# han0110/learn-fhe

Measured on AMD Instinct MI355X. Metric: NTTs/sec at N=2^14 q~60-bit, higher is better.
Workload: dtype u64

## Files before the change

### learn-fhe_amd/csrc/arith.hpp

```cpp
#pragma once
#include <type_traits>

#include "dev_arith.hpp"

namespace fhe {

#define FHE_GLOBAL __attribute__((address_space(1)))
template <class T>
__device__ __forceinline__ const FHE_GLOBAL T *as_global(const T *p) {
    return (const FHE_GLOBAL T *)p;
}
#define FHE_CONST __attribute__((address_space(4)))
template <class T>
__device__ __forceinline__ const FHE_CONST T *as_const(const T *p) {
    return (const FHE_CONST T *)p;
}

#define FHE_HEADER_KERNEL static __attribute__((unused)) __global__

template <int I, int END, typename F>
__device__ __forceinline__ void static_for(F &&f) {
    if constexpr (I < END) {
        f(std::integral_constant<int, I>{});
        static_for<I + 1, END>(f);
    }
}

struct ModDesc {
    u64 q;
    const TwPair *tw, *twi;
    u64 ninv[20], ninv_s[20];
    u64 ninv_w[20], ninv_w_s[20];
    u64 one_s;
    const u64 *tww, *twwi;
    unsigned pm_c;
    int pm_b;
    const uint4 *twd, *twdi;
    unsigned ds_pow;
    uint4 ds_ninv[20], ds_ninv_w[20], ds_one;
    const uint4 *twd3i;
    unsigned twd3_stride;
    u64 bar_mu;
    int bar_sh1, bar_sh2;
};

struct NttIo {
    const u64 *src = nullptr;
    unsigned src_mod = 1;
    const u64 *mul = nullptr;
    unsigned mul_div = 1, mul_period = 1;
    const u64 *src2 = nullptr, *src3 = nullptr, *src4 = nullptr;
    unsigned src_group = 0;
    u64 *dst2 = nullptr;
    unsigned dst_period = 0, dst_first2 = 0;
};
__device__ __forceinline__ const u64 *ntt_src(const NttIo &io, unsigned sub, int log_len, const u64 *own) {
    if (!io.src) return own;
    if (io.src_group) {
        const unsigned gsel = sub / io.src_group, r = sub - gsel * io.src_group;
        const u64 *b = gsel == 0 ? io.src : gsel == 1 ? io.src2 : gsel == 2 ? io.src3 : io.src4;
        return b + (size_t(r) << log_len);
    }
    return io.src + (size_t(sub % io.src_mod) << log_len);
}

struct ArithShoup {
    typedef u64 Elem;
    struct K {
        u64 q, q2;
        const FHE_CONST TwPair *tw, *twi;
        u64 ninv, ninv_s;
        int pb, prefix;
        TwPair ninv_w;
        Barrett bar;
    };
    static __device__ __forceinline__ K make(const ModDesc &D, int log_n_total, int pb, int prefix) {
        return K{D.q, 2 * D.q, as_const(D.tw), as_const(D.twi), pb ? 1 : D.ninv[log_n_total], pb ? D.one_s : D.ninv_s[log_n_total], pb, prefix,
                 TwPair{D.ninv_w[log_n_total], D.ninv_w_s[log_n_total]}, Barrett{D.q, D.bar_mu, D.bar_sh1, D.bar_sh2}};
    }
    static __device__ __forceinline__ u64 mulvar(u64 x, u64 y, const K &k) { return mulmod_barrett(x, y, k.bar); }
    template <int PH = 1>
    static __device__ __forceinline__ void gs_last_scaled(u64 &X, u64 &Y, const K &k) {
        const u64 s = X + Y, d = X - Y + k.q2;
        X = csub(mul_shoup_lazy(s, k.ninv, k.ninv_s, k.q), k.q);
        Y = csub(mul_shoup_lazy(d, k.ninv_w.w, k.ninv_w.ws, k.q), k.q);
    }
    template <int PH = 1>
    static __device__ __forceinline__ void gs_last_plain(u64 &X, u64 &Y, const TwPair &p, const K &k) {
        gs_bfly(X, Y, p.w, p.ws, k.q, k.q2);
        X = csub(X, k.q); Y = csub(Y, k.q);
    }
    typedef TwPair TwRaw;
    typedef TwPair TwReg;
    static constexpr int PREFETCH = 0;
    template <bool INV>
    static __device__ __forceinline__ TwRaw fetch(const K &k, int idx) {
        const FHE_CONST TwPair *p = (INV ? k.twi : k.tw) + idx;
// ... 390 lines not shown
        u128 b[32] = {};
        for (int r = 0; r < 32; ++r) b[r] = s.diag.out[r & 7];
        x32(b);
        int g = 3;
        for (int l = 3; l >= 0; --l) layer(s, b, g++, 4, l, 2, 16, false);
        x21(b);
        for (int l = 3; l >= 0; --l) layer(s, b, g++, 4, l, 2, 16, false);
        if (!x10(b, R0, pairs)) s.ok = false;
        for (int l = R0 - 1; l >= 1; --l) layer(s, b, g++, R0, l, 32 >> R0, 1 << R0, false);
        layer(s, b, g++, R0, 0, 32 >> R0, 1 << R0, true);
        s.layers = g;
        return s;
    }
    template <int R0, bool PAIRS, int IN>
    static constexpr Sched SCHED = make(R0, PAIRS, IN);
    template <int R0, bool PAIRS, int IN> static constexpr bool fx(int g, int o) { return SCHED<R0, PAIRS, IN>.lay[g - 3][o].fx; }
    template <int R0, bool PAIRS, int IN> static constexpr bool fy(int g, int o) { return SCHED<R0, PAIRS, IN>.lay[g - 3][o].fy; }
    template <int R0, bool PAIRS, int IN> static constexpr bool fs(int g, int o) { return SCHED<R0, PAIRS, IN>.lay[g - 3][o].fs; }
    template <int R0, bool PAIRS, int IN> static constexpr int mi(int g, int o) {
        return SCHED<R0, PAIRS, IN>.mi(SCHED<R0, PAIRS, IN>.lay[g - 3][o].m);
    }
    template <int R0, bool PAIRS, int IN> static constexpr bool valid() {
        constexpr Sched s = SCHED<R0, PAIRS, IN>;
        return s.ok && s.layers == 11 + R0 && s.bflies == 16 * (11 + R0);
    }
    template <int R0, bool PAIRS, int IN> static constexpr int folds_x100() { return SCHED<R0, PAIRS, IN>.folds * 100 / SCHED<R0, PAIRS, IN>.bflies; }

    static_assert(keep_ok(RMAX), "a raw product must be able to enter a butterfly as it stands");
    static_assert(fold_max(CAP - 1) < 2 * QMIN, "a folded value is below 2q: one conditional subtraction makes it canonical");
    static_assert(cover(RMAX) == L::K, "the offset of a raw subtrahend is DsLazy's K");
    static_assert(valid<1, true, 0>() && valid<2, true, 0>() && valid<3, true, 0>() && valid<4, false, 0>(), "whole rings, canonical inputs");
    static_assert(valid<1, true, 1>() && valid<2, true, 1>() && valid<3, true, 1>() && valid<4, false, 1>(), "multiplied inputs");
    static_assert(valid<1, false, 0>() && valid<2, false, 0>() && valid<3, false, 0>() && valid<3, false, 1>(), "the 8-byte dealing");
};
static_assert(DsGsLazy<60>::SCHED<3, true, 0>.diag.folds == 3 && DsGsLazy<60>::folds_x100<3, true, 0>() <= 75, "60 bits");
static_assert(DsGsLazy<60>::folds_x100<3, true, 1>() <= 75 && DsGsLazy<60>::folds_x100<4, false, 0>() <= 75, "60 bits");
static_assert(DsGsLazy<55>::SCHED<3, true, 0>.diag.folds == 0 && DsGsLazy<55>::folds_x100<3, true, 0>() <= 30, "55 bits");
static_assert(DsGsLazy<54>::SCHED<3, true, 0>.diag.folds == 0 && DsGsLazy<54>::folds_x100<3, true, 0>() <= 30, "54 bits");

template <int B>
struct ArithDS {
    typedef u64 Elem;
    static constexpr u64 MASK = (u64(1) << B) - 1;
    static constexpr int SPLIT = B - 31;
    typedef uint4 TwRaw;
    typedef uint4 TwReg;
    struct K {
        DsK m;
        const FHE_CONST uint4 *tw, *twi;
        uint4 ninv, ninv_w;
        int pb, prefix;
        const FHE_CONST uint4 *tw3i;
        unsigned tw3_stride;
    };
    static constexpr int PREFETCH = 4;
    static __host__ __device__ __forceinline__ uint4 split(u64 w, u64 q) {
        const u64 w1 = (u64)((((unsigned __int128)w) << 32) % q);
        const u64 lo = (u64(1) << SPLIT) - 1;
        return uint4{(unsigned)(w & lo), (unsigned)(w >> SPLIT), (unsigned)(w1 & lo), (unsigned)(w1 >> SPLIT)};
    }
    template <bool INV>
    static __device__ __forceinline__ TwRaw fetch(const K &k, int idx) {
        const FHE_CONST uint4 *p = (INV ? k.twi : k.tw) + idx;
        TwRaw r;
        r.x = p->x; r.y = p->y; r.z = p->z; r.w = p->w;
        return r;
    }
    static __device__ __forceinline__ TwReg prep(const TwRaw &r) { return r; }
    static __device__ __forceinline__ K make(const ModDesc &D, int log_n_total, int pb, int prefix) {
        K k;
        k.m.q = D.q; k.m.q2 = 2 * D.q; k.m.q4 = 4 * D.q;
        k.m.c = D.pm_c; k.m.c2 = 2 * D.pm_c; k.m.pw = D.ds_pow;
        k.m.qk = Lazy::K * D.q;
        asm("" : "+s"(k.m.qk));
        k.tw = as_const(D.twd); k.twi = as_const(D.twdi);
        k.ninv = pb ? D.ds_one : D.ds_ninv[log_n_total];
        k.ninv_w = D.ds_ninv_w[log_n_total];
        k.pb = pb; k.prefix = prefix;
        k.tw3i = as_const(D.twd3i); k.tw3_stride = D.twd3_stride;
        return k;
    }
    typedef DsLazy<B> Lazy;
    static __host__ __device__ __forceinline__ u64 mul_raw(u64 y, const uint4 &w, const DsK &m, u64 add = 0) {
        const unsigned y0 = (unsigned)y, y1 = (unsigned)(y >> 32);
        const u64 s1 = (u64)w.y * y0 + (u64)w.w * y1;
        const u64 s0 = ((u64)w.x * y0 + add) + (u64)w.z * y1;
        const u64 v = (u64)(unsigned)s1 * m.pw + s0;
        return (u64)(unsigned)(s1 >> 32) * m.c2 + v;
    }
    static __host__ __device__ __forceinline__ u64 fold1(u64 x, const DsK &m) {
        const unsigned hi = (unsigned)(x >> 32), h = hi >> (B - 32);
        const u64 base = ((u64)(hi & (unsigned)(MASK >> 32)) << 32) | (unsigned)x;
        return (u64)h * m.c + base;
    }
    static __device__ __forceinline__ u64 mul(u64 y, const uint4 &w, const DsK &m) { return fold1(mul_raw(y, w, m), m); }
    static __device__ __forceinline__ u64 mulvar(u64 x, u64 y, const K &k) {
        return pm_mul<B>(x, ArithPM<B>::split(y), PmK{k.m.q, k.m.q2, k.m.q4, k.m.c, k.m.c2});
    }
    static __device__ __forceinline__ void ct(u64 &X, u64 &Y, const TwReg &w, const K &k) {
        const u64 t = mul(Y, w, k.m);
        const u64 x = X;
        X = x + t;
        Y = x + k.m.q2 - t;
    }
    template <bool FOLDX>
    static __host__ __device__ __forceinline__ void ct_lazy(u64 &X, u64 &Y, const TwReg &w, const DsK &m) {
        const u64 x = FOLDX ? fold1(X, m) : X;
        const u64 r = mul_raw(Y, w, m, x);
        X = r;
        Y = ((x << 1) + m.qk) - r;
    }
    static constexpr int CT_LAYERS = 64;
    static constexpr bool PASS_FOLD = false;
    static constexpr int CT_SPAN = B >= 64 - 2 ? 1 : (((1 << (64 - B)) - 2) / 2 > 64 ? 64 : ((1 << (64 - B)) - 2) / 2);
    static __device__ constexpr bool ct_fold_at(int layer) { return layer > 0 && layer % CT_SPAN == 0; }
    template <int PH>
    static __device__ __forceinline__ void gs(u64 &X, u64 &Y, const TwReg &w, const K &k) {
        static_assert(PH < 64 - B - 1, "sums overflow");
        const u64 s = X + Y;
        const u64 d = X + (k.m.q2 << PH) - Y;
        X = s;
        Y = mul(d, w, k.m);
    }
    static constexpr bool GS_FOLDS = true;
    static constexpr int GS_SPAN = 64 - B - 1 > 8 ? 8 : 64 - B - 1;
    template <int PH = 1>
    static __device__ __forceinline__ void gs_last_scaled(u64 &X, u64 &Y, const K &k) {
        const u64 s = X + Y, d = X + (k.m.q2 << PH) - Y;
        X = csub(mul(s, k.ninv, k.m), k.m.q);
        Y = csub(mul(d, k.ninv_w, k.m), k.m.q);
    }
    template <int PH = 1>
// ... 52 lines not shown
        v[4] = mul_raw((u0 + ou2) - u2, e[3], m); used(3, v[4]);
        v[5] = mul_raw((u1 + ou3) - u3, e[4], m); used(4, v[5]);
        v[6] = mul_raw((e0 + orr) - e2, e[5], m); used(5, v[6]);
        v[7] = mul_raw((e1 + orr) - e3, e[6], m); used(6, v[7]);
    }
    typedef typename ArithPM<B>::MacAcc MacAcc;
    static constexpr int MAC_TERMS = ArithPM<B>::MAC_TERMS;
    static __device__ __forceinline__ PmK pmk(const K &k) { return PmK{k.m.q, k.m.q2, k.m.q4, k.m.c, k.m.c2}; }
    static __device__ __forceinline__ MacAcc mac_zero() { return MacAcc{0, 0}; }
    static __device__ __forceinline__ u64 mac_in(u64 x, const K &) { return x; }
    static __device__ __forceinline__ MacAcc mac(MacAcc acc, u64 xin, u64 kval, int term, const K &k, const Barrett &) {
        const unsigned wl = (unsigned)kval;
        const PmTw w{wl, wl << (63 - B), (unsigned)(kval >> 32)};
        u64 v, u;
        pm_mul_vu<B>(xin, w, v, u);
        acc.v += v; acc.u += u;
        if ((term % MAC_TERMS) == MAC_TERMS - 1) acc = MacAcc{pm_reduce_vu<B>(acc.v, acc.u, pmk(k)), 0};
        return acc;
    }
    static __device__ __forceinline__ u64 mac_finish(MacAcc acc, const K &k) { return pm_reduce_vu<B>(acc.v, acc.u, pmk(k)); }
};

#define FHE_SCHED_FENCE() asm volatile("" ::: "memory")

template <int L0_, int R_, int l_, int REP0_, int NREP_, int STRIDE_, bool SHARED_, int REP_SHIFT_ = 0>
struct Unit {
    static constexpr int L0 = L0_, R = R_, l = l_, REP0 = REP0_, NREP = NREP_, STRIDE = STRIDE_, REP_SHIFT = REP_SHIFT_;
    static constexpr bool SHARED = SHARED_;
    static constexpr int NT = (SHARED_ ? 1 : NREP_) << l_;
    static constexpr int half = 1 << (R_ - 1 - l_);
};

#ifdef FHE_LAB_ABLATE
template <class A, class = void> struct tw_skip_mask { static constexpr unsigned value = 0; };
template <class A> struct tw_skip_mask<A, decltype((void)A::SKIP_MASK)> { static constexpr unsigned value = A::SKIP_MASK; };
#endif

template <class A, bool INV, class U, int NTW>
__device__ __forceinline__ void tw_load(typename A::TwRaw (&raw)[NTW], int top, const typename A::K &k) {
    static_assert(U::NT <= NTW, "twiddle buffer too small for this unit");
#pragma unroll
    for (int rr = 0; rr < (U::SHARED ? 1 : U::NREP); ++rr)
#pragma unroll
        for (int b = 0; b < (1 << U::l); ++b) {
            const int tp = U::SHARED ? top : (top | ((U::REP0 + rr) << U::REP_SHIFT));
            const int idx = (1 << (U::L0 + U::l + k.pb)) + ((((k.prefix << U::L0) | tp)) << U::l) + b;
#ifdef FHE_LAB_ABLATE
            if constexpr ((tw_skip_mask<A>::value >> (U::L0 + U::l)) & 1) { raw[(rr << U::l) | b] = A::fake(k, idx); continue; }
#endif
            raw[(rr << U::l) | b] = A::template fetch<INV>(k, idx);
        }
}

template <class A, class U, int NTW, int E>
__device__ __forceinline__ void ct_apply(typename A::Elem (&x)[E], const typename A::TwRaw (&raw)[NTW], const typename A::K &k) {
    if constexpr ((U::l > 0 && U::l % A::CT_LAYERS == 0) || A::ct_fold_at(U::L0 + U::l)) {
#pragma unroll
        for (int rr = 0; rr < U::NREP; ++rr)
#pragma unroll
            for (int r = 0; r < (1 << U::R); ++r) x[(U::REP0 + rr) * U::STRIDE + r] = A::fold(x[(U::REP0 + rr) * U::STRIDE + r], k);
    }
    if constexpr (U::SHARED) {
#pragma unroll
        for (int b = 0; b < (1 << U::l); ++b) {
            const typename A::TwReg w = A::prep(raw[b]);
#pragma unroll
            for (int rr = 0; rr < U::NREP; ++rr)
#pragma unroll
                for (int j = 0; j < U::half; ++j) {
                    const int o = (U::REP0 + rr) * U::STRIDE + b * 2 * U::half + j;
                    A::ct(x[o], x[o + U::half], w, k);
                }
        }
    } else {
#pragma unroll
        for (int rr = 0; rr < U::NREP; ++rr)
#pragma unroll
            for (int b = 0; b < (1 << U::l); ++b) {
                const typename A::TwReg w = A::prep(raw[(rr << U::l) | b]);
#pragma unroll
                for (int j = 0; j < U::half; ++j) {
                    const int o = (U::REP0 + rr) * U::STRIDE + b * 2 * U::half + j;
                    A::ct(x[o], x[o + U::half], w, k);
                }
            }
    }
}

template <class A, class U, int NTW, int E>
__device__ __forceinline__ void ct_apply_lazy(typename A::Elem (&x)[E], const typename A::TwRaw (&raw)[NTW], const typename A::K &k) {
    constexpr bool FOLDX = A::Lazy::fold_before(U::L0 + U::l);
    constexpr int LAZY_GROUP = 4;
    static_for<0, (U::SHARED ? (1 << U::l) : U::NREP)>([&](auto oc) {
        constexpr int outer = decltype(oc)::value;
        static_for<0, (U::SHARED ? U::NREP : (1 << U::l))>([&](auto ic) {
            constexpr int inner = decltype(ic)::value;
            constexpr int b = U::SHARED ? outer : inner, rr = U::SHARED ? inner : outer;
            const typename A::TwReg w = A::prep(raw[U::SHARED ? b : ((rr << U::l) | b)]);
#pragma unroll
            for (int j = 0; j < U::half; ++j) {
                const int o = (U::REP0 + rr) * U::STRIDE + b * 2 * U::half + j;
                A::template ct_lazy<FOLDX>(x[o], x[o + U::half], w, k.m);
                if ((j + 1) % LAZY_GROUP == 0 || j + 1 == U::half) __builtin_amdgcn_sched_barrier(0);
            }
        });
    });
// ... 78 lines not shown
```

### learn-fhe_amd/csrc/ctx.hpp

```cpp
#pragma once
#include <hip/hip_runtime.h>

#include <cstdint>
#include <vector>

#include "dev_arith.hpp"
#include "modmath.hpp"
#include "ntt_kernels.hpp"

struct fhe_ctx {
    uint64_t q = 0;
    int s = 0;
    uint64_t g = 0;
    uint64_t omega = 0;
    int log_cap = 0;
    std::vector<uint64_t> tw, twi;
    uint64_t ninv[32] = {0}, ninv_s[32] = {0};
    uint64_t ninv_w[32] = {0}, ninv_w_s[32] = {0};
    fhe::Barrett barrett{};
    int device = -1;
    fhe::TwPair *d_tw = nullptr, *d_twi = nullptr;
    u64 *d_tww = nullptr, *d_twwi = nullptr;
    uint4 *d_twd = nullptr, *d_twdi = nullptr;
    uint4 *d_twd3i = nullptr;
    int pm_b = 0;
    unsigned pm_c = 0;
    fhe::ModDesc *d_desc = nullptr;
    fhe::ModDesc h_desc{};
};

namespace fhe {
constexpr int MAX_LOG_N = 17;
int ctx_build_host(uint64_t q, fhe_ctx *c);
int ntt_fwd_multi(const ModDesc *descs, unsigned n_desc, u64 *a, int log_n, size_t batch, hipStream_t st, int pm = 0, NttIo io = NttIo());
int ntt_inv_multi(const ModDesc *descs, unsigned n_desc, u64 *a, int log_n, size_t batch, hipStream_t st, int pm = 0, NttIo io = NttIo());
int ntt_mul_multi(const ModDesc *descs, unsigned n_desc, u64 *a, int log_n, size_t batch, hipStream_t st, int pm, NttIo io);
int ntt_fwd_inner15(const ModDesc *descs, unsigned n_desc, u64 *a, size_t batch, hipStream_t st, int pm, NttIo io = NttIo());
int ntt_inv_inner15(const ModDesc *descs, unsigned n_desc, u64 *a, size_t batch, hipStream_t st, int pm, NttIo io = NttIo());
}
```

### learn-fhe_amd/csrc/ntt14w.hpp

```cpp
#pragma once
#include <type_traits>
#include "ntt_kernels.hpp"

namespace fhe {
namespace w14 {

constexpr int WSLOTS = 1088;
template <int R0> constexpr int threads() { return 64 << R0; }
template <int R0> constexpr size_t lds_bytes() { return (size_t(1) << R0) * WSLOTS * 8; }
constexpr int THREADS = threads<3>();
constexpr size_t LDS_BYTES = lds_bytes<3>();

__device__ __forceinline__ void wave_sync() {
    __builtin_amdgcn_wave_barrier();
    asm volatile("" ::: "memory");
}

template <class A, class = void> struct w14_old_deal { static constexpr bool value = false; };
template <class A> struct w14_old_deal<A, decltype((void)A::W14_OLD_DEAL)> { static constexpr bool value = true; };
template <class A, int R0>
__device__ __host__ constexpr bool w14_pairs() {
    return R0 <= 3 && !w14_old_deal<A>::value;
}

// ... 179 lines not shown
    for (int h = 0; h < 2; ++h) {
#pragma unroll
        for (int r4 = 0; r4 < 16; ++r4) wp[4 * r4] = x[((r4 & 1) << 4) | (h << 3) | (r4 >> 1)];
        wave_sync();
#pragma unroll
        for (int n4 = 0; n4 < 16; ++n4) y[(h << 4) | n4] = rp[68 * n4];
        wave_sync();
    }
#pragma unroll
    for (int r = 0; r < 32; ++r) x[r] = y[r];
}

__device__ __forceinline__ void xchg_23(u64 (&x)[32], int lane, u64 *wl) {
    const int hi5 = ((lane >> 4) << 3) | ((lane & 3) << 1) | ((lane >> 3) & 1);
    u64 *wp = wl + 34 * hi5 + ((lane >> 2) & 1);
    const u64 *rp = wl + 34 * (lane >> 5) + 2 * (lane & 15) + ((lane >> 4) & 1);
    u64 y[32];
#pragma unroll
    for (int h = 0; h < 2; ++h) {
#pragma unroll
        for (int c = 0; c < 16; ++c) wp[2 * c] = x[(h << 4) | c];
        wave_sync();
#pragma unroll
        for (int R = 0; R < 16; ++R)
            y[((R >> 2) << 3) | (h << 2) | (R & 3)] = rp[68 * R];
        wave_sync();
    }
#pragma unroll
    for (int r = 0; r < 32; ++r) x[r] = y[r];
}

__device__ __forceinline__ void xchg_32(u64 (&x)[32], int lane, u64 *wl) {
    const u64 *rp = wl + 17 * lane;
    u64 *wp = wl + 68 * (lane >> 4) + (lane & 15);
    u64 y[32];
#pragma unroll
    for (int h = 0; h < 2; ++h) {
#pragma unroll
        for (int R = 0; R < 16; ++R) wp[17 * (((R >> 2) << 4) | (R & 3))] = x[((R >> 2) << 3) | (h << 2) | (R & 3)];
        wave_sync();
#pragma unroll
        for (int c = 0; c < 16; ++c) y[(h << 4) | c] = rp[c];
        wave_sync();
    }
#pragma unroll
    for (int r = 0; r < 32; ++r) x[r] = y[r];
}

template <int R0, int l> using P0 = Unit<0, R0, l, 0, (32 >> R0), (1 << R0), true>;
template <int R0, int l> using P1 = Unit<R0, 4, l, 0, 2, 16, true>;
template <int R0, int l> using P2 = Unit<R0 + 4, 4, l, 0, 2, 16, true>;
template <int R0, int l, int AB> using P3 = Unit<R0 + 8, 3, l, AB, 1, 8, false, 6>;

template <class A>
__device__ __host__ constexpr bool w14_p3_refill() {
    return std::is_same<typename A::TwRaw, uint4>::value;
}

template <class A>
struct Tw7 {
    typename A::TwRaw l0[1], l1[2], l2[4];
};
template <class A, bool INV, int R0, int AB>
__device__ __forceinline__ void tw7_load(Tw7<A> &b, int t3, const typename A::K &k) {
    tw_load<A, INV, P3<R0, 0, AB>>(b.l0, t3, k);
    tw_load<A, INV, P3<R0, 1, AB>>(b.l1, t3, k);
    tw_load<A, INV, P3<R0, 2, AB>>(b.l2, t3, k);
}

template <int R0, bool PAIRS>
__device__ __forceinline__ void load_p0(u64 (&x)[32], const u64 *__restrict__ g, int t) {
#pragma unroll
    for (int r = 0; r < 32; ++r) {
        const int n = r & ((1 << R0) - 1), pass = r >> R0;
        if constexpr (PAIRS) {
            if (pass & 1) continue;
            const ulonglong2 v = *reinterpret_cast<const ulonglong2 *>(g + ((n << 11) | ((pass >> 1) << (7 + R0)) | (t << 1)));
            x[r] = v.x; x[r + (1 << R0)] = v.y;
        } else {
            x[r] = g[(n << 11) | (pass << (6 + R0)) | t];
        }
    }
}
template <int AB>
__device__ __forceinline__ void load_p3(u64 (&x)[32], const u64 *__restrict__ src) {
#pragma unroll
    for (int j = 0; j < 8; j += 2) {
        const ulonglong2 v = *reinterpret_cast<const ulonglong2 *>(src + (AB << 9) + j);
        x[AB * 8 + j] = v.x; x[AB * 8 + j + 1] = v.y;
    }
}
template <class A, int AB>
__device__ __forceinline__ void load_mul_p3(u64 (&x)[32], const u64 *__restrict__ src, const u64 *__restrict__ mul, const typename A::K &k) {
#pragma unroll
    for (int j = 0; j < 8; j += 2) {
        const ulonglong2 v = *reinterpret_cast<const ulonglong2 *>(src + (AB << 9) + j);
        const ulonglong2 m = *reinterpret_cast<const ulonglong2 *>(mul + (AB << 9) + j);
        x[AB * 8 + j] = A::mulvar(v.x, m.x, k); x[AB * 8 + j + 1] = A::mulvar(v.y, m.y, k);
    }
}

template <class A, int AB>
__device__ __forceinline__ void store_p3(u64 (&x)[32], u64 *__restrict__ dst_wave, int lane, u64 *wl, const typename A::K &k) {
    ulonglong2 *wr = reinterpret_cast<ulonglong2 *>(wl + 8 * lane + (lane & ~1));
    const ulonglong2 *rd = reinterpret_cast<const ulonglong2 *>(wl + 2 * lane + 2 * (lane >> 3));
#pragma unroll
    for (int j = 0; j < 4; ++j) {
        ulonglong2 v;
        v.x = A::canon_fwd(x[AB * 8 + 2 * j], k);
        v.y = A::canon_fwd(x[AB * 8 + 2 * j + 1], k);
        wr[j] = v;
    }
    wave_sync();
#pragma unroll
    for (int kk = 0; kk < 4; ++kk) {
        const ulonglong2 v = rd[72 * kk];
        x[AB * 8 + 2 * kk] = v.x; x[AB * 8 + 2 * kk + 1] = v.y;
    }
    wave_sync();
#pragma unroll
    for (int kk = 0; kk < 4; ++kk) {
        ulonglong2 v;
        v.x = x[AB * 8 + 2 * kk]; v.y = x[AB * 8 + 2 * kk + 1];
        *reinterpret_cast<ulonglong2 *>(dst_wave + (AB << 9) + 128 * kk + 2 * lane) = v;
    }
}

template <class A, int R0, bool KEEP = false>
__device__ __forceinline__ void fwd_one(u64 (&x)[32], u64 *__restrict__ g, const typename A::K &k, u64 *lds, u64 *wl,
                                        const int t, const int lane, const int w STAMP_ENTRY_PARAM) {
    typedef typename A::TwRaw Tw;
    constexpr bool LAZY = w14_lazy_fwd<A, KEEP>();
    if constexpr (LAZY) static_assert(A::Lazy::canon_ok(11 + R0), "lazy outputs of this many layers do not fit canon_fwd");
    STAMP_DECL;
    STAMP_REAL(10);
    STAMP(0);
    {
        Tw a0[1], a1[2], a2[4], a3[8];
        tw_load<A, false, P0<R0, 0>>(a0, 0, k);
        if constexpr (R0 >= 2) tw_load<A, false, P0<R0, (R0 >= 2 ? 1 : 0)>>(a1, 0, k);
        if constexpr (R0 >= 3) tw_load<A, false, P0<R0, (R0 >= 3 ? 2 : 0)>>(a2, 0, k);
        if constexpr (R0 == 4) tw_load<A, false, P0<R0, (R0 == 4 ? 3 : 0)>>(a3, 0, k);
        STAMP(1);
        FHE_SCHED_FENCE();
        w14_ct<LAZY, A, P0<R0, 0>>(x, a0, k);
        if constexpr (R0 >= 2) {
            FHE_SCHED_FENCE();
            w14_ct<LAZY, A, P0<R0, (R0 >= 2 ? 1 : 0)>>(x, a1, k);
        }
        if constexpr (R0 >= 3) {
            FHE_SCHED_FENCE();
            w14_ct<LAZY, A, P0<R0, (R0 >= 3 ? 2 : 0)>>(x, a2, k);
        }
        if constexpr (R0 == 4) {
            FHE_SCHED_FENCE();
            w14_ct<LAZY, A, P0<R0, (R0 == 4 ? 3 : 0)>>(x, a3, k);
        }
    }
    FHE_SCHED_FENCE();
    Tw b0[1], b1[2], b2[4], b3[8];
    tw_load<A, false, P1<R0, 0>>(b0, w, k); tw_load<A, false, P1<R0, 1>>(b1, w, k); tw_load<A, false, P1<R0, 2>>(b2, w, k); tw_load<A, false, P1<R0, 3>>(b3, w, k);
    STAMP(2);
    xchg_01<R0, w14_pairs<A, R0>()>(x, t, w, lds);
    STAMP(3);
    if constexpr (A::PASS_FOLD) {
#pragma unroll
        for (int r = 0; r < 32; ++r) x[r] = A::fold(x[r], k);
    }
    FHE_SCHED_FENCE();
    w14_ct<LAZY, A, P1<R0, 0>>(x, b0, k);
    FHE_SCHED_FENCE();
    w14_ct<LAZY, A, P1<R0, 1>>(x, b1, k);
    FHE_SCHED_FENCE();
    w14_ct<LAZY, A, P1<R0, 2>>(x, b2, k);
    FHE_SCHED_FENCE();
    w14_ct<LAZY, A, P1<R0, 3>>(x, b3, k);
    FHE_SCHED_FENCE();
    const int t2 = (w << 4) | (lane >> 2), t3e = (w << 8) | lane;
    Tw c0[1], c1[2], c2[4], c3[8];
    tw_load<A, false, P2<R0, 0>>(c0, t2, k); tw_load<A, false, P2<R0, 1>>(c1, t2, k); tw_load<A, false, P2<R0, 2>>(c2, t2, k);
    STAMP(4);
    xchg_12(x, lane, wl);
    STAMP(5);
    if constexpr (A::PASS_FOLD) {
#pragma unroll
        for (int r = 0; r < 32; ++r) x[r] = A::fold(x[r], k);
    }
    FHE_SCHED_FENCE();
    w14_ct<LAZY, A, P2<R0, 0>>(x, c0, k);
    FHE_SCHED_FENCE();
    w14_ct<LAZY, A, P2<R0, 1>>(x, c1, k);
    FHE_SCHED_FENCE();
    tw_load<A, false, P2<R0, 3>>(c3, t2, k);
    w14_ct<LAZY, A, P2<R0, 2>>(x, c2, k);
    FHE_SCHED_FENCE();
    w14_ct<LAZY, A, P2<R0, 3>>(x, c3, k);
    FHE_SCHED_FENCE();
    int lane3 = lane, t3 = t3e;
    if constexpr (LAZY) {
        lane3 = __builtin_amdgcn_mbcnt_hi(~0u, __builtin_amdgcn_mbcnt_lo(~0u, 0u));
        asm volatile("" : "+v"(lane3));
        t3 = (w << 8) | lane3;
    }
    Tw7<A> d[2];
    tw7_load<A, false, R0, 0>(d[0], t3, k);
    STAMP(6);
    xchg_23(x, lane3, wl);
    STAMP(7);
    if constexpr (A::PASS_FOLD) {
#pragma unroll
        for (int r = 0; r < 32; ++r) x[r] = A::fold(x[r], k);
    }
    u64 *dst_wave = g + (w << 11);
    static_for<0, 4>([&](auto abc) {
        constexpr int ab = decltype(abc)::value;
        FHE_SCHED_FENCE();
        w14_ct<LAZY, A, P3<R0, 0, ab>>(x, d[ab & 1].l0, k);
        w14_ct<LAZY, A, P3<R0, 1, ab>>(x, d[ab & 1].l1, k);
        FHE_SCHED_FENCE();
        if constexpr (ab < 3) tw7_load<A, false, R0, (ab < 3 ? ab + 1 : 3)>(d[(ab + 1) & 1], t3, k);
        w14_ct<LAZY, A, P3<R0, 2, ab>>(x, d[ab & 1].l2, k);
        FHE_SCHED_FENCE();
        if constexpr (KEEP) {
#pragma unroll
            for (int j = 0; j < 8; ++j) x[ab * 8 + j] = A::canon_fwd(x[ab * 8 + j], k);
        } else {
            store_p3<A, ab>(x, dst_wave, lane3, wl, k);
        }
    });
    STAMP(8);
#ifdef NTT14_STAMPS
    asm volatile("s_waitcnt vmcnt(0)" ::: "memory");
#endif
    STAMP(9);
    STAMP_REAL(11);
    STAMP_FLUSH();
}

template <class A>
__device__ __host__ constexpr bool w14_p3_diag() {
    return std::is_same<typename A::TwRaw, uint4>::value;
}

template <class A, int R0, int AB>
__device__ __forceinline__ int p3_blk(int t3, const typename A::K &k) {
    return (1 << (R0 + 8 + k.pb)) + ((k.prefix << (R0 + 8)) | t3 | (AB << 6));
}
template <class A, int R0, int AB>
__device__ __forceinline__ void p3_diag_load(uint4 (&e)[7], int t3, const typename A::K &k) {
    const int blk = p3_blk<A, R0, AB>(t3, k);
#pragma unroll
    for (int p = 0; p < 7; ++p) {
        const FHE_CONST uint4 *q = k.tw3i + size_t(p) * k.tw3_stride + blk;
        e[p] = uint4{q->x, q->y, q->z, q->w};
    }
}
template <class A, int R0, int AB, int NEXT>
__device__ __forceinline__ void p3_diag_apply(u64 (&x)[32], uint4 (&e)[7], const uint4 &ci, const uint4 &cj, const uint4 &cij, int t3,
                                              const typename A::K &k) {
    const auto &m = k.m;
    u64 *v = x + 8 * AB;
    const u64 s0 = v[0] + v[1], t0 = v[0] + m.q2 - v[1];
    const u64 s1 = v[2] + v[3], t1 = A::mul(v[2] + m.q2 - v[3], ci, m);
    const u64 s2 = v[4] + v[5], t2 = A::mul(v[4] + m.q2 - v[5], cj, m);
    const u64 s3 = v[6] + v[7], t3v = A::mul(v[6] + m.q2 - v[7], cij, m);
    const u64 u0 = s0 + s1, e0 = s0 + m.q4 - s1;
    const u64 u1 = t0 + t1, e1 = t0 + m.q2 - t1;
    const u64 u2 = s2 + s3, e2 = A::mul(s2 + m.q4 - s3, ci, m);
    const u64 u3 = t2 + t3v, e3 = A::mul(t2 + m.q2 - t3v, ci, m);
    const int blk = NEXT >= 0 ? p3_blk<A, R0, (NEXT >= 0 ? NEXT : 0)>(t3, k) : 0;
    auto refill = [&](int p) {
        if constexpr (NEXT >= 0) {
            const FHE_CONST uint4 *q = k.tw3i + size_t(p) * k.tw3_stride + blk;
// ... 30 lines not shown
    if constexpr (LZ) p3_diag_apply_lazy<A, SEL, R0, AB, NEXT>(x, e, ci, cj, cij, t3, k, off);
    else p3_diag_apply<A, R0, AB, NEXT>(x, e, ci, cj, cij, t3, k);
}

template <class A, bool PFX, int R0, int IN, bool LZ>
__device__ __forceinline__ void inv_one(u64 (&x)[32], Tw7<A> (&d)[2], u64 *__restrict__ g, const typename A::K &k, u64 *lds, u64 *wl,
                                        const int t, const int lane, const int w STAMP_ENTRY_PARAM) {
    typedef typename A::TwRaw Tw;
    int t2 = 0;
    if constexpr (!LZ) t2 = (w << 4) | (lane >> 2);
    const int t3 = (w << 8) | lane;
    typedef GsSel<R0, w14_pairs<A, R0>(), IN> SEL;
    u64 off[W14_OFFS] = {};
    if constexpr (LZ) {
        static_assert(w14_p3_diag<A>(), "the lazy inverse is written for the diagonal form of pass 3");
        static_assert(A::GsLazy::template valid<R0, w14_pairs<A, R0>(), IN>(), "no valid lazy schedule");
        w14_gs_offs<A, SEL>(off, k);
    }
    STAMP_DECL;
    STAMP_REAL(10);
    STAMP(0);
    constexpr bool REFILL = w14_p3_refill<A>();
    Tw c3[8], c2[4], c1[2], c0[1];
    if constexpr (w14_p3_diag<A>()) {
        uint4(&e)[7] = reinterpret_cast<uint4(&)[7]>(d[0]);
        const uint4 ci = A::template fetch<true>(k, 1), cj = A::template fetch<true>(k, 2), cij = A::template fetch<true>(k, 3);
        FHE_SCHED_FENCE();
        w14_p3<LZ, A, SEL, R0, 0, 1>(x, e, ci, cj, cij, t3, k, off);
        FHE_SCHED_FENCE();
        w14_p3<LZ, A, SEL, R0, 1, 2>(x, e, ci, cj, cij, t3, k, off);
        FHE_SCHED_FENCE();
        w14_p3<LZ, A, SEL, R0, 2, 3>(x, e, ci, cj, cij, t3, k, off);
        FHE_SCHED_FENCE();
        w14_p3<LZ, A, SEL, R0, 3, -1>(x, e, ci, cj, cij, t3, k, off);
    } else
    static_for<0, 4>([&](auto abc) {
        constexpr int ab = decltype(abc)::value, nx = ab < 3 ? ab + 1 : 3;
        Tw7<A> &e = d[REFILL ? 0 : ab & 1];
        FHE_SCHED_FENCE();
        gs_apply<A, P3<R0, 2, ab>, 0>(x, e.l2, k);
        if constexpr (REFILL && ab < 3) tw_load<A, true, P3<R0, 2, nx>>(e.l2, t3, k);
        FHE_SCHED_FENCE();
        gs_apply<A, P3<R0, 1, ab>, 1>(x, e.l1, k);
        if constexpr (REFILL && ab < 3) tw_load<A, true, P3<R0, 1, nx>>(e.l1, t3, k);
        gs_apply<A, P3<R0, 0, ab>, 2>(x, e.l0, k);
        if constexpr (REFILL && ab < 3) tw_load<A, true, P3<R0, 0, nx>>(e.l0, t3, k);
        FHE_SCHED_FENCE();
        if constexpr (!REFILL && ab < 2) tw7_load<A, true, R0, (ab < 2 ? ab + 2 : 3)>(d[ab & 1], t3, k);
    });
    FHE_SCHED_FENCE();
    STAMP(1);
    if constexpr (LZ) t2 = (w << 4) | (lane >> 2);
    constexpr bool C3_LATE = sizeof(Tw) > 8;
    if constexpr (!C3_LATE) tw_load<A, true, P2<R0, 3>>(c3, t2, k);
    xchg_32(x, lane, wl);
    STAMP(2);
    FHE_SCHED_FENCE();
    if constexpr (C3_LATE) tw_load<A, true, P2<R0, 3>>(c3, t2, k);
    constexpr bool C2_LATE = LZ;
    if constexpr (!C2_LATE) tw_load<A, true, P2<R0, 2>>(c2, t2, k);
    if constexpr (LZ) w14_gs_offs<A, SEL>(off, k);
    w14_gs<LZ, A, P2<R0, 3>, SEL, 3>(x, c3, k, off);
    FHE_SCHED_FENCE();
    if constexpr (C2_LATE) tw_load<A, true, P2<R0, 2>>(c2, t2, k);
    tw_load<A, true, P2<R0, 1>>(c1, t2, k); tw_load<A, true, P2<R0, 0>>(c0, t2, k);
    w14_gs<LZ, A, P2<R0, 2>, SEL, 4>(x, c2, k, off);
    FHE_SCHED_FENCE();
    w14_gs<LZ, A, P2<R0, 1>, SEL, 5>(x, c1, k, off);
    FHE_SCHED_FENCE();
    w14_gs<LZ, A, P2<R0, 0>, SEL, 6>(x, c0, k, off);
    FHE_SCHED_FENCE();
    STAMP(3);
    Tw b3[8], b2[4], b1[2], b0[1];
    tw_load<A, true, P1<R0, 3>>(b3, w, k); tw_load<A, true, P1<R0, 2>>(b2, w, k); tw_load<A, true, P1<R0, 1>>(b1, w, k); tw_load<A, true, P1<R0, 0>>(b0, w, k);
    xchg_21(x, lane, wl);
    STAMP(4);
    FHE_SCHED_FENCE();
    if constexpr (LZ) w14_gs_offs<A, SEL>(off, k);
    w14_gs<LZ, A, P1<R0, 3>, SEL, 7>(x, b3, k, off);
    FHE_SCHED_FENCE();
    w14_gs<LZ, A, P1<R0, 2>, SEL, 8>(x, b2, k, off);
    FHE_SCHED_FENCE();
    w14_gs<LZ, A, P1<R0, 1>, SEL, 9>(x, b1, k, off);
    FHE_SCHED_FENCE();
    w14_gs<LZ, A, P1<R0, 0>, SEL, 10>(x, b0, k, off);
    FHE_SCHED_FENCE();
    STAMP(5);
    Tw a3[8], a2[4], a1[2], a0[1];
    if constexpr (R0 == 4) tw_load<A, true, P0<R0, (R0 == 4 ? 3 : 0)>>(a3, 0, k);
    if constexpr (R0 >= 3) tw_load<A, true, P0<R0, (R0 >= 3 ? 2 : 0)>>(a2, 0, k);
    if constexpr (R0 >= 2) tw_load<A, true, P0<R0, (R0 >= 2 ? 1 : 0)>>(a1, 0, k);
    if constexpr (PFX) tw_load<A, true, P0<R0, 0>>(a0, 0, k);
    xchg_10<R0, w14_pairs<A, R0>()>(x, t, w, lds);
    STAMP(6);
    if constexpr (LZ) w14_gs_offs<A, SEL>(off, k);
    if constexpr (R0 == 4) {
        FHE_SCHED_FENCE();
        w14_gs<LZ, A, P0<R0, (R0 == 4 ? 3 : 0)>, SEL, 11>(x, a3, k, off);
    }
    if constexpr (R0 >= 3) {
        FHE_SCHED_FENCE();
        w14_gs<LZ, A, P0<R0, (R0 >= 3 ? 2 : 0)>, SEL, 8 + R0>(x, a2, k, off);
    }
    if constexpr (R0 >= 2) {
        FHE_SCHED_FENCE();
        w14_gs<LZ, A, P0<R0, (R0 >= 2 ? 1 : 0)>, SEL, 9 + R0>(x, a1, k, off);
    }
    STAMP(7);
    typename A::TwReg wlast{};
    if constexpr (PFX) wlast = A::prep(a0[0]);
    constexpr int LAST_PH = A::GS_SPAN > 0 ? (10 + R0) % (A::GS_SPAN > 0 ? A::GS_SPAN : 1) : 1;
    constexpr int HALF = 1 << (R0 - 1), REPS = 32 >> R0, CH = HALF < 4 ? HALF : 4;
    constexpr bool PAIRS = w14_pairs<A, R0>();
    constexpr int CHP = CH < 2 ? 1 : CH / 2;
    if constexpr (LZ) {
        w14_gs_offs<A, SEL>(off, k);
        auto last = [&](auto oc) {
            typedef typename A::GsLazy G;
// ... 199 lines not shown
```

### learn-fhe_amd/csrc/ring_api.hip

```cpp
#include <hip/hip_runtime.h>
#include <cstdlib>

#include <cstring>
#include <mutex>
#include <new>
#include <set>
#include <utility>

#include "../../include/fhe_ring.h"
#include "api_common.hpp"
#include "ctx.hpp"
#include "dispatch.hpp"
#include "ntt_kernels.hpp"
#include "ntt14w.hpp"

using fhe::u64;

namespace {
int check_transform(const fhe_ctx *ctx, const void *a, size_t n, size_t batch) {
    if (!ctx || !is_pow2(n) || (!a && batch)) return FHE_ERR_INVALID;
    if (n == 1) return FHE_OK;
    int log_n = ilog2(n);
    if (log_n > ctx->s - 1) return FHE_ERR_NO_ROOT;
    if (log_n > ctx->log_cap) return FHE_ERR_UNSUPPORTED;
// ... 227 lines not shown
    if (!c) return FHE_ERR_INVALID;
    int rc = fhe::ctx_build_host(q, c);
    if (rc != FHE_OK) { delete c; return rc; }
    c->device = device;
    if (device >= 0) {
        DeviceGuard guard(device);
        if (!guard.ok) { delete c; return FHE_ERR_HIP; }
        const size_t cap = c->tw.size();
        std::vector<fhe::TwPair> pf(cap), pi(cap);
        for (size_t j = 0; j < cap; ++j) {
            pf[j] = {c->tw[j], fhe::shoup(c->tw[j], q)};
            pi[j] = {c->twi[j], fhe::shoup(c->twi[j], q)};
        }
        hipError_t e = hipMalloc(&c->d_tw, cap * sizeof(fhe::TwPair));
        if (e == hipSuccess) e = hipMalloc(&c->d_twi, cap * sizeof(fhe::TwPair));
        if (e == hipSuccess) e = hipMemcpy(c->d_tw, pf.data(), cap * sizeof(fhe::TwPair), hipMemcpyHostToDevice);
        if (e == hipSuccess) e = hipMemcpy(c->d_twi, pi.data(), cap * sizeof(fhe::TwPair), hipMemcpyHostToDevice);
        if (e == hipSuccess && c->pm_b) {
            const int b = c->pm_b;
            std::vector<uint64_t> lf(cap), li(cap);
            auto pack = [b](uint64_t w) { return ((w >> (b - 31)) << 32) | (w & ((uint64_t(1) << (b - 31)) - 1)); };
            for (size_t j = 0; j < cap; ++j) { lf[j] = pack(c->tw[j]); li[j] = pack(c->twi[j]); }
            e = hipMalloc((void **)&c->d_tww, 2 * cap * sizeof(uint64_t));
            c->d_twwi = c->d_tww + cap;
            if (e == hipSuccess) e = hipMemcpy(c->d_tww, lf.data(), cap * sizeof(uint64_t), hipMemcpyHostToDevice);
            if (e == hipSuccess) e = hipMemcpy(c->d_twwi, li.data(), cap * sizeof(uint64_t), hipMemcpyHostToDevice);
        }
        if (e == hipSuccess && c->pm_b) {
            const int b = c->pm_b;
            std::vector<uint4> df(cap), di(cap);
            auto split = [b, q](uint64_t w) {
                const uint64_t w1 = (uint64_t)((((unsigned __int128)w) << 32) % q), lo = (uint64_t(1) << (b - 31)) - 1;
                return uint4{(unsigned)(w & lo), (unsigned)(w >> (b - 31)), (unsigned)(w1 & lo), (unsigned)(w1 >> (b - 31))};
            };
            for (size_t j = 0; j < cap; ++j) { df[j] = split(c->tw[j]); di[j] = split(c->twi[j]); }
            for (int k = 0; k < 20; ++k) { c->h_desc.ds_ninv[k] = split(c->ninv[k]); c->h_desc.ds_ninv_w[k] = split(c->ninv_w[k]); }
            c->h_desc.ds_one = split(1);
            e = hipMalloc((void **)&c->d_twd, 2 * cap * sizeof(uint4));
            c->d_twdi = c->d_twd + cap;
            if (e == hipSuccess) e = hipMemcpy(c->d_twd, df.data(), cap * sizeof(uint4), hipMemcpyHostToDevice);
            if (e == hipSuccess) e = hipMemcpy(c->d_twdi, di.data(), cap * sizeof(uint4), hipMemcpyHostToDevice);
            if (e == hipSuccess && cap >= 8) {
                const size_t stride = cap / 4;
                std::vector<uint4> d3(7 * stride, uint4{0, 0, 0, 0});
                for (size_t blk = 1; blk < stride; ++blk) {
                    const uint64_t th = c->twi[4 * blk];
                    uint64_t pw = th;
                    for (int p = 0; p < 7; ++p) { d3[p * stride + blk] = split(pw); pw = fhe::mulmod(pw, th, q); }
                }
                e = hipMalloc((void **)&c->d_twd3i, d3.size() * sizeof(uint4));
                if (e == hipSuccess) e = hipMemcpy(c->d_twd3i, d3.data(), d3.size() * sizeof(uint4), hipMemcpyHostToDevice);
                c->h_desc.twd3i = c->d_twd3i; c->h_desc.twd3_stride = (unsigned)stride;
            }
        }
        c->h_desc.tww = c->d_tww;
        c->h_desc.twwi = c->d_twwi;
        c->h_desc.twd = c->d_twd;
        c->h_desc.twdi = c->d_twdi;
        c->h_desc.ds_pow = c->pm_b ? 1u << (c->pm_b - 31) : 0;
        c->h_desc.pm_b = c->pm_b;
        c->h_desc.pm_c = c->pm_c;
        c->h_desc.q = q;
        c->h_desc.tw = c->d_tw;
        c->h_desc.twi = c->d_twi;
        for (int k = 0; k < 20; ++k) {
            c->h_desc.ninv[k] = c->ninv[k]; c->h_desc.ninv_s[k] = c->ninv_s[k];
            c->h_desc.ninv_w[k] = c->ninv_w[k]; c->h_desc.ninv_w_s[k] = c->ninv_w_s[k];
        }
        c->h_desc.one_s = fhe::shoup(1, q);
        c->h_desc.bar_mu = c->barrett.mu; c->h_desc.bar_sh1 = c->barrett.sh1; c->h_desc.bar_sh2 = c->barrett.sh2;
        if (e == hipSuccess) e = hipMalloc(&c->d_desc, sizeof(fhe::ModDesc));
        if (e == hipSuccess) e = hipMemcpy(c->d_desc, &c->h_desc, sizeof(fhe::ModDesc), hipMemcpyHostToDevice);
        if (e != hipSuccess) {
            g_last_hip = (int)e;
            fhe_ctx_destroy(c);
            return FHE_ERR_HIP;
        }
    }
    *out = c;
    return FHE_OK;
}

void fhe_ctx_destroy(fhe_ctx *c) {
    if (!c) return;
    if (c->device >= 0) {
        DeviceGuard guard(c->device);
        if (c->d_tw) (void)hipFree(c->d_tw);
        if (c->d_twi) (void)hipFree(c->d_twi);
        if (c->d_desc) (void)hipFree(c->d_desc);
        if (c->d_tww) (void)hipFree(c->d_tww);
        if (c->d_twd) (void)hipFree(c->d_twd);
        if (c->d_twd3i) (void)hipFree(c->d_twd3i);
    }
    delete c;
}

int fhe_ctx_info(const fhe_ctx *c, uint64_t *q, int *s, uint64_t *g, uint64_t *omega) {
    if (!c) return FHE_ERR_INVALID;
    if (q) *q = c->q;
    if (s) *s = c->s;
    if (g) *g = c->g;
    if (omega) *omega = c->omega;
    return FHE_OK;
}

int fhe_ctx_twiddles(const fhe_ctx *c, int inverse, uint64_t *out, size_t count) {
    if (!c || !out) return FHE_ERR_INVALID;
    const auto &t = inverse ? c->twi : c->tw;
    if (count > t.size()) return FHE_ERR_UNSUPPORTED;
    std::memcpy(out, t.data(), count * sizeof(uint64_t));
    return FHE_OK;
}

static int transform_entry(const fhe_ctx *ctx, uint64_t *a, size_t n, size_t batch, fhe_mem mem, void *stream, bool inverse) {
    int rc = check_transform(ctx, a, n, batch);
    if (rc != FHE_OK) return rc;
    if (ctx->device < 0) return FHE_ERR_NO_DEVICE;
    if (n == 1 || batch == 0) return FHE_OK;
    if (batch > 0xffffffffull) return FHE_ERR_UNSUPPORTED;
    hipStream_t st = (hipStream_t)stream;
    DeviceGuard guard(ctx->device);
    if (!guard.ok) return FHE_ERR_HIP;
    Mirror m(a, n * batch, mem, true, st);
    if (m.rc != FHE_OK) return m.rc;
    rc = inverse ? fhe::ntt_inv_device(ctx, m.d, ilog2(n), batch, st) : fhe::ntt_fwd_device(ctx, m.d, ilog2(n), batch, st);
    if (rc != FHE_OK) return rc;
    return m.sync_out(st);
}

int fhe_ntt_fwd(const fhe_ctx *ctx, uint64_t *a, size_t n, size_t batch, fhe_mem mem, void *stream) {
    return transform_entry(ctx, a, n, batch, mem, stream, false);
}

int fhe_ntt_inv(const fhe_ctx *ctx, uint64_t *a, size_t n, size_t batch, fhe_mem mem, void *stream) {
    return transform_entry(ctx, a, n, batch, mem, stream, true);
}

static int launch_pointwise(const fhe_ctx *ctx, u64 *a, const u64 *b, size_t len, hipStream_t st) {
    return fhe::launch<fhe::pointwise_mul_kernel>(grid_for(len, 4096), 256, 0, st, a, b, len, ctx->barrett);
}

int fhe_pointwise_mul(const fhe_ctx *ctx, uint64_t *a, const uint64_t *b, size_t len, fhe_mem mem, void *stream) {
    if (!ctx || ((!a || !b) && len)) return FHE_ERR_INVALID;
    if (ctx->device < 0) return FHE_ERR_NO_DEVICE;
    if (len == 0) return FHE_OK;
// ... 81 lines not shown
```

Baseline: 15.97 million.

## Add lane-contiguous transposed twiddle table for forward pass-3 loads

Builds a transposed copy of the forward split twiddles so that, for layers 1–2 inside a unit, consecutive lanes read consecutive 16-byte entries. Loads go through raw buffer instructions with a bounds-checked resource. It is enabled only for the forward pass-3 site by default, aiming for coalesced twiddle fetches instead of strided scalar/constant reads. It adds table memory and setup cost, and the inverse sites are disabled because only forward copies are filled.

Result: no change. 16.07 million (median of 6 runs) (+0.6%).

```diff
diff --git a/learn-fhe_amd/csrc/arith.hpp b/learn-fhe_amd/csrc/arith.hpp
--- a/learn-fhe_amd/csrc/arith.hpp
+++ b/learn-fhe_amd/csrc/arith.hpp
@@ -40,9 +40,24 @@
     uint4 ds_ninv[20], ds_ninv_w[20], ds_one;
     const uint4 *twd3i;
     unsigned twd3_stride;
+    const uint4 *twdt;
+    unsigned twdt_stride, twdt_entries;
     u64 bar_mu;
     int bar_sh1, bar_sh2;
 };
+
+constexpr int TWDT_COPIES = 3;
+__host__ __device__ constexpr size_t twdt_index(size_t cap, int l, int L, unsigned j, size_t T) {
+    return size_t(l - 1) * cap + (size_t(1) << L) + (size_t(j) << (L - l)) + T;
+}
+template <class E>
+inline void twdt_fill(E *dst, const E *src, int log_cap, int copies = TWDT_COPIES) {
+    const size_t cap = size_t(1) << log_cap;
+    for (int l = 1; l <= copies; ++l)
+        for (int L = l; L < log_cap; ++L)
+            for (size_t T = 0; T < (size_t(1) << (L - l)); ++T)
+                for (unsigned j = 0; j < (1u << l); ++j) dst[twdt_index(cap, l, L, j, T)] = src[(size_t(1) << L) + (T << l) + j];
+}
 
 struct NttIo {
     const u64 *src = nullptr;
@@ -539,6 +554,8 @@
         int pb, prefix;
         const FHE_CONST uint4 *tw3i;
         unsigned tw3_stride;
+        const uint4 *twt;
+        unsigned twt_cap, twt_entries;
     };
     static constexpr int PREFETCH = 4;
     static __host__ __device__ __forceinline__ uint4 split(u64 w, u64 q) {
@@ -565,6 +582,7 @@
         k.ninv_w = D.ds_ninv_w[log_n_total];
         k.pb = pb; k.prefix = prefix;
         k.tw3i = as_const(D.twd3i); k.tw3_stride = D.twd3_stride;
+        k.twt = D.twdt; k.twt_cap = D.twdt_stride; k.twt_entries = D.twdt_entries;
         return k;
     }
     typedef DsLazy<B> Lazy;
@@ -723,6 +741,25 @@
         }
 }
 
+template <class A, bool INV, class U, int NTW>
+__device__ __forceinline__ void tw_load_t(uint4 (&raw)[NTW], int top, const typename A::K &k) {
+    static_assert(U::NT <= NTW, "twiddle buffer too small for this unit");
+    static_assert(U::l >= 1 && U::l <= TWDT_COPIES, "no lane-contiguous copy for this layer");
+    typedef unsigned v4u __attribute__((ext_vector_type(4)));
+    const int L = U::L0 + U::l + k.pb;
+    const auto rsrc = __builtin_amdgcn_make_buffer_rsrc(const_cast<uint4 *>(k.twt), 0, int(16u * k.twt_entries), 0x00020000);
+    const unsigned voff = unsigned(top) << 4;
+#pragma unroll
+    for (int rr = 0; rr < (U::SHARED ? 1 : U::NREP); ++rr)
+#pragma unroll
+        for (int b = 0; b < (1 << U::l); ++b) {
+            const unsigned rep = U::SHARED ? 0u : unsigned(U::REP0 + rr) << U::REP_SHIFT;
+            const size_t e = twdt_index(k.twt_cap, U::l, L, b, (size_t(k.prefix) << U::L0) + rep) + (INV ? size_t(TWDT_COPIES) * k.twt_cap : 0);
+            const v4u v = __builtin_amdgcn_raw_buffer_load_b128(rsrc, voff, unsigned(e) << 4, 0);
+            raw[(rr << U::l) | b] = uint4{v.x, v.y, v.z, v.w};
+        }
+}
+
 template <class A, class U, int NTW, int E>
 __device__ __forceinline__ void ct_apply(typename A::Elem (&x)[E], const typename A::TwRaw (&raw)[NTW], const typename A::K &k) {
     if constexpr ((U::l > 0 && U::l % A::CT_LAYERS == 0) || A::ct_fold_at(U::L0 + U::l)) {
diff --git a/learn-fhe_amd/csrc/ctx.hpp b/learn-fhe_amd/csrc/ctx.hpp
--- a/learn-fhe_amd/csrc/ctx.hpp
+++ b/learn-fhe_amd/csrc/ctx.hpp
@@ -23,6 +23,7 @@
     u64 *d_tww = nullptr, *d_twwi = nullptr;
     uint4 *d_twd = nullptr, *d_twdi = nullptr;
     uint4 *d_twd3i = nullptr;
+    uint4 *d_twdt = nullptr;
     int pm_b = 0;
     unsigned pm_c = 0;
     fhe::ModDesc *d_desc = nullptr;
diff --git a/learn-fhe_amd/csrc/ntt14w.hpp b/learn-fhe_amd/csrc/ntt14w.hpp
--- a/learn-fhe_amd/csrc/ntt14w.hpp
+++ b/learn-fhe_amd/csrc/ntt14w.hpp
@@ -255,6 +255,27 @@
 template <int R0, int l> using P2 = Unit<R0 + 4, 4, l, 0, 2, 16, true>;
 template <int R0, int l, int AB> using P3 = Unit<R0 + 8, 3, l, AB, 1, 8, false, 6>;
 
+constexpr unsigned TWT_FWD3 = 1, TWT_FWD2 = 2, TWT_INV2 = 4;
+constexpr unsigned W14_TWT_SITES = TWT_FWD3;
+template <class A, class = void> struct w14_twt_sites { static constexpr unsigned value = W14_TWT_SITES; };
+template <class A> struct w14_twt_sites<A, decltype((void)A::W14_TWT_SITES)> { static constexpr unsigned value = A::W14_TWT_SITES; };
+template <unsigned SITE, class A>
+__device__ __host__ constexpr bool w14_twt_on() {
+    return std::is_same<typename A::TwRaw, uint4>::value && (w14_twt_sites<A>::value & SITE) != 0;
+}
+template <unsigned SITE, class A, bool INV, class U, int NTW>
+__device__ __forceinline__ void w14_tw(typename A::TwRaw (&raw)[NTW], int top, const typename A::K &k) {
+#ifdef FHE_LAB_ABLATE
+    constexpr bool LOADED = ((tw_skip_mask<A>::value >> (U::L0 + U::l)) & 1) == 0;
+#else
+    constexpr bool LOADED = true;
+#endif
+    if constexpr (w14_twt_on<SITE, A>() && U::l >= 1 && LOADED)
+        tw_load_t<A, INV, U>(raw, top, k);
+    else
+        tw_load<A, INV, U>(raw, top, k);
+}
+
 template <class A>
 __device__ __host__ constexpr bool w14_p3_refill() {
     return std::is_same<typename A::TwRaw, uint4>::value;
@@ -264,11 +285,11 @@
 struct Tw7 {
     typename A::TwRaw l0[1], l1[2], l2[4];
 };
-template <class A, bool INV, int R0, int AB>
+template <class A, bool INV, int R0, int AB, unsigned SITE = 0>
 __device__ __forceinline__ void tw7_load(Tw7<A> &b, int t3, const typename A::K &k) {
     tw_load<A, INV, P3<R0, 0, AB>>(b.l0, t3, k);
-    tw_load<A, INV, P3<R0, 1, AB>>(b.l1, t3, k);
-    tw_load<A, INV, P3<R0, 2, AB>>(b.l2, t3, k);
+    w14_tw<SITE, A, INV, P3<R0, 1, AB>>(b.l1, t3, k);
+    w14_tw<SITE, A, INV, P3<R0, 2, AB>>(b.l2, t3, k);
 }
 
 template <int R0, bool PAIRS>
@@ -335,6 +356,7 @@
     typedef typename A::TwRaw Tw;
     constexpr bool LAZY = w14_lazy_fwd<A, KEEP>();
     if constexpr (LAZY) static_assert(A::Lazy::canon_ok(11 + R0), "lazy outputs of this many layers do not fit canon_fwd");
+    constexpr unsigned S2 = KEEP ? 0u : TWT_FWD2, S3 = KEEP ? 0u : TWT_FWD3;
     STAMP_DECL;
     STAMP_REAL(10);
     STAMP(0);
@@ -381,7 +403,7 @@
     FHE_SCHED_FENCE();
     const int t2 = (w << 4) | (lane >> 2), t3e = (w << 8) | lane;
     Tw c0[1], c1[2], c2[4], c3[8];
-    tw_load<A, false, P2<R0, 0>>(c0, t2, k); tw_load<A, false, P2<R0, 1>>(c1, t2, k); tw_load<A, false, P2<R0, 2>>(c2, t2, k);
+    tw_load<A, false, P2<R0, 0>>(c0, t2, k); w14_tw<S2, A, false, P2<R0, 1>>(c1, t2, k); w14_tw<S2, A, false, P2<R0, 2>>(c2, t2, k);
     STAMP(4);
     xchg_12(x, lane, wl);
     STAMP(5);
@@ -394,7 +416,7 @@
     FHE_SCHED_FENCE();
     w14_ct<LAZY, A, P2<R0, 1>>(x, c1, k);
     FHE_SCHED_FENCE();
-    tw_load<A, false, P2<R0, 3>>(c3, t2, k);
+    w14_tw<S2, A, false, P2<R0, 3>>(c3, t2, k);
     w14_ct<LAZY, A, P2<R0, 2>>(x, c2, k);
     FHE_SCHED_FENCE();
     w14_ct<LAZY, A, P2<R0, 3>>(x, c3, k);
@@ -406,7 +428,7 @@
         t3 = (w << 8) | lane3;
     }
     Tw7<A> d[2];
-    tw7_load<A, false, R0, 0>(d[0], t3, k);
+    tw7_load<A, false, R0, 0, S3>(d[0], t3, k);
     STAMP(6);
     xchg_23(x, lane3, wl);
     STAMP(7);
@@ -421,7 +443,7 @@
         w14_ct<LAZY, A, P3<R0, 0, ab>>(x, d[ab & 1].l0, k);
         w14_ct<LAZY, A, P3<R0, 1, ab>>(x, d[ab & 1].l1, k);
         FHE_SCHED_FENCE();
-        if constexpr (ab < 3) tw7_load<A, false, R0, (ab < 3 ? ab + 1 : 3)>(d[(ab + 1) & 1], t3, k);
+        if constexpr (ab < 3) tw7_load<A, false, R0, (ab < 3 ? ab + 1 : 3), S3>(d[(ab + 1) & 1], t3, k);
         w14_ct<LAZY, A, P3<R0, 2, ab>>(x, d[ab & 1].l2, k);
         FHE_SCHED_FENCE();
         if constexpr (KEEP) {
@@ -558,18 +580,18 @@
     STAMP(1);
     if constexpr (LZ) t2 = (w << 4) | (lane >> 2);
     constexpr bool C3_LATE = sizeof(Tw) > 8;
-    if constexpr (!C3_LATE) tw_load<A, true, P2<R0, 3>>(c3, t2, k);
+    if constexpr (!C3_LATE) w14_tw<TWT_INV2, A, true, P2<R0, 3>>(c3, t2, k);
     xchg_32(x, lane, wl);
     STAMP(2);
     FHE_SCHED_FENCE();
-    if constexpr (C3_LATE) tw_load<A, true, P2<R0, 3>>(c3, t2, k);
+    if constexpr (C3_LATE) w14_tw<TWT_INV2, A, true, P2<R0, 3>>(c3, t2, k);
     constexpr bool C2_LATE = LZ;
-    if constexpr (!C2_LATE) tw_load<A, true, P2<R0, 2>>(c2, t2, k);
+    if constexpr (!C2_LATE) w14_tw<TWT_INV2, A, true, P2<R0, 2>>(c2, t2, k);
     if constexpr (LZ) w14_gs_offs<A, SEL>(off, k);
     w14_gs<LZ, A, P2<R0, 3>, SEL, 3>(x, c3, k, off);
     FHE_SCHED_FENCE();
-    if constexpr (C2_LATE) tw_load<A, true, P2<R0, 2>>(c2, t2, k);
-    tw_load<A, true, P2<R0, 1>>(c1, t2, k); tw_load<A, true, P2<R0, 0>>(c0, t2, k);
+    if constexpr (C2_LATE) w14_tw<TWT_INV2, A, true, P2<R0, 2>>(c2, t2, k);
+    w14_tw<TWT_INV2, A, true, P2<R0, 1>>(c1, t2, k); tw_load<A, true, P2<R0, 0>>(c0, t2, k);
     w14_gs<LZ, A, P2<R0, 2>, SEL, 4>(x, c2, k, off);
     FHE_SCHED_FENCE();
     w14_gs<LZ, A, P2<R0, 1>, SEL, 5>(x, c1, k, off);
diff --git a/learn-fhe_amd/csrc/ring_api.hip b/learn-fhe_amd/csrc/ring_api.hip
--- a/learn-fhe_amd/csrc/ring_api.hip
+++ b/learn-fhe_amd/csrc/ring_api.hip
@@ -303,6 +303,13 @@
                 if (e == hipSuccess) e = hipMemcpy(c->d_twd3i, d3.data(), d3.size() * sizeof(uint4), hipMemcpyHostToDevice);
                 c->h_desc.twd3i = c->d_twd3i; c->h_desc.twd3_stride = (unsigned)stride;
             }
+            if (e == hipSuccess && cap >= 2) {
+                std::vector<uint4> dt(2 * cap, uint4{0, 0, 0, 0});
+                fhe::twdt_fill(dt.data(), df.data(), c->log_cap, 2);
+                e = hipMalloc((void **)&c->d_twdt, dt.size() * sizeof(uint4));
+                if (e == hipSuccess) e = hipMemcpy(c->d_twdt, dt.data(), dt.size() * sizeof(uint4), hipMemcpyHostToDevice);
+                c->h_desc.twdt = c->d_twdt; c->h_desc.twdt_stride = (unsigned)cap; c->h_desc.twdt_entries = (unsigned)dt.size();
+            }
         }
         c->h_desc.tww = c->d_tww;
         c->h_desc.twwi = c->d_twwi;
@@ -342,6 +349,7 @@
         if (c->d_tww) (void)hipFree(c->d_tww);
         if (c->d_twd) (void)hipFree(c->d_twd);
         if (c->d_twd3i) (void)hipFree(c->d_twd3i);
+        if (c->d_twdt) (void)hipFree(c->d_twdt);
     }
     delete c;
 }
```
